# SnakeOnex/vit-is-all-you-need

Hardware: AMD Instinct MI355X
Metric: images/sec ViT-B/16 224px bf16 fwd+bwd (higher is better)
Workload: dtype bf16; 1 GPU; ViT-B/16 224x224 bf16 forward+loss+backward, batch 256 per GPU (BASELINE configs[1]; configs[2] at 8 GPUs), random-init weights, 197 tokens, 79.44 M params; global_batch=256, parallelism=dp1

## Files before the change

### vit-is-all-you-need_amd/csrc/gemm_nt_ld.h

```cpp
#pragma once
#include "gemm_nt_seam.h"

namespace {

template <int EPI, bool TAB = false, int SCHED = 1>
__global__ __launch_bounds__(768) void gemm_nt_ld_kernel(const GemmNtArgs p) {
  static_assert(EPI == EPI_BIAS_BF16 || EPI == EPI_GELU || EPI == EPI_DGELU || EPI == EPI_DGELU_NOCS, "epilogues of the loader form");
  static_assert(SCHED == 1, "request schedule");
  static_assert(!TAB || EPI == EPI_GELU, "table = GELU");
  constexpr bool DG = EPI == EPI_DGELU || EPI == EPI_DGELU_NOCS;
  constexpr bool CS = EPI == EPI_DGELU;
  constexpr int BM = 256, BN = 256, MT = 8, NT = 4;
  constexpr int AREG = 16384, ABUF = 32768, BBUF = 32768, BBASE = 2 * ABUF, OPS = BBASE + 2 * BBUF;
  constexpr int STG = 2048, TABOFF = OPS + 8 * STG;
  constexpr unsigned OOB = 0x80000000u;

  extern __shared__ __attribute__((aligned(16))) char smem[];
  const int tid = threadIdx.x, lane = tid & 63;
  const int wave = __builtin_amdgcn_readfirstlane(tid >> 6);
  const int tiles_n = (p.N + BN - 1) / BN, tiles_m = (p.M + BM - 1) / BM;
  const int ntiles = tiles_m * tiles_n;
  const int K = p.K;
  const int nkt = K / 64;
  auto coords = [&](int ti) { return nt_tile<BM>(ti, tiles_m, tiles_n); };

  if (wave >= 8) {
    const int l = wave - 8;
    const srd_t srdA = make_srd(p.A, (size_t)p.M * K * 2);
    const srd_t srdB = make_srd(p.B, (size_t)p.N * K * 2);
    const srd_t srdBias = make_srd(p.bias ? (const void*)p.bias : p.out, p.bias ? (size_t)p.N * 4 : 0);
    const unsigned ldsA = lds_addr(smem) + l * 4096;
    const unsigned ldsB = lds_addr(smem) + BBASE + l * 8192;
    unsigned voffA[2][4], voffB[8];
    auto offsets = [&](const NtTile& t) {
      const int r8 = lane >> 3;
      const unsigned chunk = (unsigned)(((lane & 7) ^ r8) * 16);
#pragma unroll
      for (int h = 0; h < 2; ++h)
#pragma unroll
        for (int i = 0; i < 4; ++i) {
          const int a = 4 * l + i;
          const int row = min(t.m0 + (a >> 3) * 128 + h * 64 + (a & 7) * 8 + r8, p.M - 1);
          voffA[h][i] = (unsigned)row * (unsigned)(K * 2) + chunk;
        }
#pragma unroll
      for (int i = 0; i < 8; ++i) {
        const int row = min(t.n0 + (8 * l + i) * 8 + r8, p.N - 1);
        voffB[i] = (unsigned)row * (unsigned)(K * 2) + chunk;
      }
    };
    bool live = true;
    unsigned so = 0u, par = 0u;
    auto request_b = [&](int i) {
      asm_glds16(srdB, ldsB + par * BBUF + i * 1024, live ? voffB[i] : OOB, so);
    };
    auto request_a = [&](int h, int i) {
      asm_glds16(srdA, ldsA + par * ABUF + h * AREG + i * 1024, live ? voffA[h][i] : OOB, so);
    };
    auto target = [&](int kt, bool lv) {
      live = lv;
      so = live ? (unsigned)kt * 128u : 0u;
      par = (unsigned)(kt & 1);
    };
    __builtin_amdgcn_s_setprio(3);
    int ti = blockIdx.x;
    NtTile cur = coords(ti);
    offsets(cur);
    int bias_n0 = cur.n0;
    target(0, true);
#pragma unroll
    for (int i = 0; i < 8; ++i) request_b(i);
#pragma unroll
    for (int i = 0; i < 4; ++i) request_a(0, i);
#pragma unroll
    for (int i = 0; i < 4; ++i) request_a(1, i);
    VITAMD_WAIT_VM(4);
    __builtin_amdgcn_s_barrier();
    for (;;) {
      const int ti_next = ti + (int)gridDim.x;
      const bool has_next = ti_next < ntiles;
      for (int kt = 0; kt < nkt; ++kt) {
        const bool last = kt + 1 == nkt;
        if (last && has_next) {
          cur = coords(ti_next);
          offsets(cur);
        }
        target(last ? 0 : kt + 1, !last || has_next);
        request_b(0); request_b(1); request_b(2);
        __builtin_amdgcn_s_barrier();
        request_b(3); request_b(4); request_b(5);
        VITAMD_WAIT_VM(6);
        __builtin_amdgcn_s_barrier();
        if constexpr (!DG) {
          if (kt == 0) {
            asm_glds4(srdBias, lds_addr(smem) + OPS + l * STG, (unsigned)(bias_n0 + l * 64 + lane) * 4u, 0u);
            asm_glds4(srdBias, lds_addr(smem) + OPS + (4 + l) * STG, (unsigned)(bias_n0 + l * 64 + lane) * 4u, 0u);
          }
        }
        request_b(6); request_b(7); request_a(0, 0);
        __builtin_amdgcn_s_barrier();
        request_a(0, 1); request_a(0, 2); request_a(0, 3);
        __builtin_amdgcn_s_barrier();
        request_a(1, 0); request_a(1, 1);
        __builtin_amdgcn_s_barrier();
        request_a(1, 2); request_a(1, 3);
        __builtin_amdgcn_s_barrier();
        __builtin_amdgcn_s_barrier();
        VITAMD_WAIT_VM(4);
        __builtin_amdgcn_s_barrier();
      }
      __builtin_amdgcn_s_barrier();
      if (!has_next) break;
      ti = ti_next;
      bias_n0 = cur.n0;
    }
    asm volatile("s_waitcnt vmcnt(0)" ::: "memory");
    return;
  }

  const int wm = wave >> 2, wn = wave & 3;
  const srd_t rsO = make_srd(p.out, (size_t)p.M * p.ldo * 2);
  const srd_t rsO2 = make_srd(EPI == EPI_GELU ? p.out2 : p.out, (size_t)p.M * p.ldo * 2);
  const srd_t srdAux = make_srd(DG ? p.aux : p.out, (size_t)p.M * p.ldo * 2);
  if constexpr (TAB) gelu_table_to_lds(p.gelu_tab, smem + TABOFF, tid);
  __builtin_amdgcn_s_barrier();
  asm volatile("" ::: "memory");
  for (int ti = blockIdx.x; ti < ntiles; ti += (int)gridDim.x) {
    const NtTile cur = coords(ti);
    if (wm == 1) __builtin_amdgcn_s_barrier();
    f32x4 acc[MT][NT];
#pragma unroll
    for (int i = 0; i < MT; ++i)
#pragma unroll
      for (int j = 0; j < NT; ++j) acc[i][j] = (f32x4){0.f, 0.f, 0.f, 0.f};
    {
      int l2 = (int)__builtin_amdgcn_mbcnt_hi(~0u, __builtin_amdgcn_mbcnt_lo(~0u, 0u));
      asm volatile("" : "+v"(l2));
      const char *rdA[2], *rdB[2];
      frag_bases(smem + wm * 8192, l2, rdA);
      frag_bases(smem + BBASE + wn * 8192, l2, rdB);
      bf16x8 bq[NT], af[4];
      auto ktile = [&](auto bufc) {
        constexpr int BUF = decltype(bufc)::value;
#pragma unroll
        for (int ph = 0; ph < 4; ++ph) {
          const int ks = ph >> 1, h = ph & 1;
          if (h == 0) {
#pragma unroll
            for (int j = 0; j < NT; ++j) bq[j] = *(const bf16x8*)(rdB[ks] + BUF * BBUF + j * 2048);
          }
#pragma unroll
          for (int ii = 0; ii < 4; ++ii) af[ii] = *(const bf16x8*)(rdA[ks] + BUF * ABUF + h * AREG + ii * 2048);
          __builtin_amdgcn_sched_barrier(0);
          __builtin_amdgcn_s_barrier();
          asm volatile("s_waitcnt lgkmcnt(0)" ::: "memory");
          __builtin_amdgcn_sched_barrier(0);
          __builtin_amdgcn_s_setprio(1);
#pragma unroll
          for (int ii = 0; ii < 4; ++ii)
#pragma unroll
            for (int j = 0; j < NT; ++j)
              acc[4 * h + ii][j] = __builtin_amdgcn_mfma_f32_16x16x32_bf16(bq[j], af[ii], acc[4 * h + ii][j], 0, 0, 0);
          __builtin_amdgcn_s_setprio(0);
          __builtin_amdgcn_sched_barrier(0);
          __builtin_amdgcn_s_barrier();
          asm volatile("" ::: "memory");
        }
      };
      for (int kt = 0; kt < nkt; kt += 2) {
        ktile(std::integral_constant<int, 0>{});
        ktile(std::integral_constant<int, 1>{});
      }
    }
    if (wm == 0) __builtin_amdgcn_s_barrier();

    int ln = (int)__builtin_amdgcn_mbcnt_hi(~0u, __builtin_amdgcn_mbcnt_lo(~0u, 0u));
    asm volatile("" : "+v"(ln));
    const int mloc = ln & 15, g = ln >> 4, rsub = ln >> 3, pc = ln & 7;
    char* const stg = smem + OPS + wave * STG;
    const int m0 = cur.m0, n0 = cur.n0;
    const int ncol = n0 + wn * 64 + 8 * (pc ^ rsub);
    const bool ncol_ok = ncol < p.N;
    const int mrow0 = m0 + wm * 128 + rsub;
    const unsigned obase = ncol_ok ? (unsigned)mrow0 * (unsigned)(p.ldo * 2) + (unsigned)ncol * 2u : OOB;
    const unsigned rstep = (unsigned)(p.ldo * 2) * 8u;
    u32x4 aux[DG ? 2 * MT : 1];
    u32x2 pk[DG ? MT : 1][NT];
    f32x4 bias4[NT];
    if constexpr (DG) {
#pragma unroll
      for (int i = 0; i < MT; ++i)
#pragma unroll
        for (int j = 0; j < NT; ++j) pk[i][j] = (u32x2){pack_bf16x2(acc[i][j][0], acc[i][j][1]), pack_bf16x2(acc[i][j][2], acc[i][j][3])};
#pragma unroll
      for (int it = 0; it < 2 * MT; ++it) aux[it] = asm_bload16(srdAux, mrow0 + 8 * it < p.M ? obase : OOB, rstep * (unsigned)it);
      static_assert(MT == 8, "16 pre-load registers named in one asm statement");
      asm volatile("s_waitcnt vmcnt(0)" : "+v"(aux[0]), "+v"(aux[1]), "+v"(aux[2]), "+v"(aux[3]), "+v"(aux[4]), "+v"(aux[5]), "+v"(aux[6]), "+v"(aux[7]), "+v"(aux[8]), "+v"(aux[9]), "+v"(aux[10]), "+v"(aux[11]), "+v"(aux[12]), "+v"(aux[13]), "+v"(aux[14]), "+v"(aux[15]) :: "memory");
    } else {
#pragma unroll
      for (int j = 0; j < NT; ++j)
#pragma unroll
        for (int r = 0; r < 4; ++r) bias4[j][r] = round_bf16(((const float*)stg)[16 * j + 4 * g + r]);
    }
    float cs[8];
#pragma unroll
    for (int c = 0; c < 8; ++c) cs[c] = 0.f;
#pragma unroll
    for (int i = 0; i < MT; ++i) {
#pragma unroll
      for (int j = 0; j < NT; ++j) {
        u32x2 o;
        if constexpr (DG) o = pk[i][j];
        else {
          const f32x4 v = acc[i][j] + bias4[j];
          o = (u32x2){pack_bf16x2(v[0], v[1]), pack_bf16x2(v[2], v[3])};
        }
        *(u32x2*)(stg + mloc * 128 + (((2 * j + (g >> 1)) ^ (mloc & 7)) << 4) + (g & 1) * 8) = o;
      }
#pragma unroll
      for (int h = 0; h < 2; ++h) {
        const u32x4 v = *(const u32x4*)(stg + (rsub + 8 * h) * 128 + pc * 16);
        const unsigned voff = mrow0 + 16 * i + 8 * h < p.M ? obase : OOB;
        const unsigned soff = rstep * (unsigned)(2 * i + h);
        if constexpr (EPI == EPI_BIAS_BF16) {
          asm_bstore16_nt(v, rsO, voff, soff);
        } else if constexpr (EPI == EPI_GELU) {
          u32x4 a, d = v;
          if constexpr (TAB) gelu_lookup8(v, smem + TABOFF, p.gelu_dg != 0, a, d);
          else
#pragma unroll
            for (int c = 0; c < 4; ++c) {
              float dlo, dhi;
              a[c] = pack_bf16x2(gelu_fwd_grad(bf16lo(v[c]), dlo), gelu_fwd_grad(bf16hi(v[c]), dhi));
              if (p.gelu_dg) d[c] = pack_bf16x2(dlo, dhi);
            }
          asm_bstore16_nt(d, rsO, voff, soff);
          asm_bstore16_nt(a, rsO2, voff, soff);
        } else {
          const u32x4 pz = aux[2 * i + h];
          u32x4 o;
#pragma unroll
          for (int c = 0; c < 4; ++c) {
            const float lo = round_bf16(bf16lo(v[c]) * bf16lo(pz[c]));
            const float hi = round_bf16(bf16hi(v[c]) * bf16hi(pz[c]));
            if constexpr (CS) { if (voff != OOB) { cs[2 * c] += lo; cs[2 * c + 1] += hi; } }
            o[c] = pack_bf16x2(lo, hi);
          }
          asm_bstore16_nt(o, rsO, voff, soff);
        }
      }
    }
    if constexpr (CS) {
#pragma unroll
      for (int bf = 1; bf < 8; bf <<= 1)
#pragma unroll
        for (int c = 0; c < 8; ++c) cs[c] += __shfl_xor(cs[c], 9 * bf, 64);
      float s = cs[0];
#pragma unroll
      for (int c = 1; c < 8; ++c) s = rsub == c ? cs[c] : s;
      atomicAdd(p.colsum + n0 + wn * 64 + 8 * (pc ^ rsub) + rsub, s);
    }
    asm volatile("s_waitcnt lgkmcnt(0)" ::: "memory");
  }
}

template <int EPI, bool TAB = false, int SCHED = 1>
int launch_ld(const GemmNtArgs& p, hipStream_t stream, int cus) {
  if (TAB && !p.gelu_tab) return VITAMD_ERR_ARG;
  return launch_tiles(gemm_nt_ld_kernel<EPI, TAB, SCHED>, p, stream, 256, 768, 160 * 1024, cus);
}

static bool ld_ok(const GemmNtArgs& p) { return seam_ok(p) && p.K % 128 == 0; }

}
```

Baseline: 9351 images/sec.

## Prefetch dGELU epilogue factors in loader waves and hand over through LDS

For the dGELU epilogue GEMM with K=768, the loader waves now issue the aux-factor loads during the final k-tiles of the main loop, using a fully unrolled compile-time schedule. They then pass the factors to the compute waves through the freed operand LDS buffers. Previously the compute waves loaded those factors from global memory in the epilogue and stalled on vmcnt(0). The cost is extra loader registers (32 u32x4), two more barrier rounds per tile, and a ds_bpermute rewrite of the colsum shuffle.

```diff
diff --git a/vit-is-all-you-need_amd/csrc/gemm_nt_ld.h b/vit-is-all-you-need_amd/csrc/gemm_nt_ld.h
--- a/vit-is-all-you-need_amd/csrc/gemm_nt_ld.h
+++ b/vit-is-all-you-need_amd/csrc/gemm_nt_ld.h
@@ -1,15 +1,31 @@
 #pragma once
+#include <utility>
 #include "gemm_nt_seam.h"
 
 namespace {
+
+
+template <int NKT> struct NtFactorPlan {
+  static constexpr int FA = 4, FKT0 = NKT - 1 - 32 / FA;
+  static constexpr bool fetches(int kt) { return NKT > 0 && kt >= FKT0 && kt <= NKT - 2; }
+  static constexpr int it(int j) { return 8 * (j >> 4) + (j & 7); }
+  static constexpr int w(int j) { return (j >> 3) & 1; }
+  static constexpr int reg(int j) { return 16 * w(j) + it(j); }
+};
+template <int... I, class F>
+__device__ __forceinline__ void nt_static_for(std::integer_sequence<int, I...>, F&& f) { (f(std::integral_constant<int, I>{}), ...); }
 
 template <int EPI, bool TAB = false, int SCHED = 1>
 __global__ __launch_bounds__(768) void gemm_nt_ld_kernel(const GemmNtArgs p) {
   static_assert(EPI == EPI_BIAS_BF16 || EPI == EPI_GELU || EPI == EPI_DGELU || EPI == EPI_DGELU_NOCS, "epilogues of the loader form");
-  static_assert(SCHED == 1, "request schedule");
+  constexpr int NKT = SCHED == 1 ? 0 : SCHED;
   static_assert(!TAB || EPI == EPI_GELU, "table = GELU");
   constexpr bool DG = EPI == EPI_DGELU || EPI == EPI_DGELU_NOCS;
   constexpr bool CS = EPI == EPI_DGELU;
+  constexpr bool PF = NKT > 0;
+  using FP = NtFactorPlan<NKT>;
+  constexpr int FA = FP::FA, FKT0 = FP::FKT0;
+  static_assert(!PF || (DG && NKT % 2 == 0 && FKT0 >= 0), "factor-prefetch form");
   constexpr int BM = 256, BN = 256, MT = 8, NT = 4;
   constexpr int AREG = 16384, ABUF = 32768, BBUF = 32768, BBASE = 2 * ABUF, OPS = BBASE + 2 * BBUF;
   constexpr int STG = 2048, TABOFF = OPS + 8 * STG;
@@ -21,8 +37,9 @@
   const int tiles_n = (p.N + BN - 1) / BN, tiles_m = (p.M + BM - 1) / BM;
   const int ntiles = tiles_m * tiles_n;
   const int K = p.K;
-  const int nkt = K / 64;
+  const int nkt = PF ? NKT : K / 64;
   auto coords = [&](int ti) { return nt_tile<BM>(ti, tiles_m, tiles_n); };
+  auto handover = [&](int w) { return smem + (w < 4 ? ABUF : BBASE + BBUF) + (w & 3) * 8192; };
 
   if (wave >= 8) {
     const int l = wave - 8;
@@ -32,9 +49,24 @@
     const unsigned ldsA = lds_addr(smem) + l * 4096;
     const unsigned ldsB = lds_addr(smem) + BBASE + l * 8192;
     unsigned voffA[2][4], voffB[8];
+    const srd_t srdAux = make_srd(DG ? p.aux : p.out, (size_t)p.M * p.ldo * 2);
+    u32x4 fr[PF ? 32 : 1];
+    unsigned fbase = OOB;
+    int frows = 0;
     auto offsets = [&](const NtTile& t) {
-      const int r8 = lane >> 3;
-      const unsigned chunk = (unsigned)(((lane & 7) ^ r8) * 16);
+      int ln = lane;
+      if constexpr (PF) {
+        ln = (int)__builtin_amdgcn_mbcnt_hi(~0u, __builtin_amdgcn_mbcnt_lo(~0u, 0u));
+        asm volatile("" : "+v"(ln));
+      }
+      const int r8 = ln >> 3;
+      const unsigned chunk = (unsigned)(((ln & 7) ^ r8) * 16);
+      if constexpr (PF) {
+        const int mrow0 = t.m0 + (l >> 1) * 128 + r8;
+        const int ncol = t.n0 + (2 * l & 3) * 64 + 8 * ((ln & 7) ^ r8);
+        fbase = ncol < p.N ? (unsigned)mrow0 * (unsigned)(p.ldo * 2) + (unsigned)ncol * 2u : OOB;
+        frows = p.M - mrow0;
+      }
 #pragma unroll
       for (int h = 0; h < 2; ++h)
 #pragma unroll
@@ -57,6 +89,7 @@
     auto request_a = [&](int h, int i) {
       asm_glds16(srdA, ldsA + par * ABUF + h * AREG + i * 1024, live ? voffA[h][i] : OOB, so);
     };
+    const unsigned rstep = (unsigned)(p.ldo * 2) * 8u;
     auto target = [&](int kt, bool lv) {
       live = lv;
       so = live ? (unsigned)kt * 128u : 0u;
@@ -79,6 +112,7 @@
     for (;;) {
       const int ti_next = ti + (int)gridDim.x;
       const bool has_next = ti_next < ntiles;
+      if constexpr (!PF) {
       for (int kt = 0; kt < nkt; ++kt) {
         const bool last = kt + 1 == nkt;
         if (last && has_next) {
@@ -109,7 +143,60 @@
         VITAMD_WAIT_VM(4);
         __builtin_amdgcn_s_barrier();
       }
+      } else {
+        nt_static_for(std::make_integer_sequence<int, PF ? NKT : 1>{}, [&](auto ktc) {
+          constexpr int KT = decltype(ktc)::value;
+          constexpr bool last = KT + 1 == NKT;
+          if (last && has_next) {
+            cur = coords(ti_next);
+            offsets(cur);
+          }
+          target(last ? 0 : KT + 1, !last || has_next);
+          request_b(0); request_b(1); request_b(2);
+          __builtin_amdgcn_s_barrier();
+          request_b(3); request_b(4); request_b(5);
+          VITAMD_WAIT_VM(FP::fetches(KT - 1) ? 6 + FA : 6);
+          __builtin_amdgcn_s_barrier();
+          request_b(6); request_b(7); request_a(0, 0);
+          __builtin_amdgcn_s_barrier();
+          request_a(0, 1); request_a(0, 2); request_a(0, 3);
+          __builtin_amdgcn_s_barrier();
+          request_a(1, 0); request_a(1, 1);
+          __builtin_amdgcn_s_barrier();
+          request_a(1, 2); request_a(1, 3);
+          __builtin_amdgcn_s_barrier();
+          __builtin_amdgcn_s_barrier();
+          if constexpr (FP::fetches(KT - 1)) {
+            constexpr int J = (KT - 1 - FKT0) * FA;
+            static_assert(FA == 4, "four factor registers named in one asm statement");
+            asm volatile("s_waitcnt vmcnt(4)" : "+v"(fr[FP::reg(J)]), "+v"(fr[FP::reg(J + 1)]), "+v"(fr[FP::reg(J + 2)]), "+v"(fr[FP::reg(J + 3)]) :: "memory");
+          } else {
+            VITAMD_WAIT_VM(4);
+          }
+          if constexpr (FP::fetches(KT)) {
+#pragma unroll
+            for (int a = 0; a < FA; ++a) {
+              const int j = (KT - FKT0) * FA + a, it = FP::it(j), w = FP::w(j);
+              fr[FP::reg(j)] = asm_bload16(srdAux, 8 * it < frows ? fbase : OOB, rstep * (unsigned)it + 128u * (unsigned)w);
+            }
+          }
+          __builtin_amdgcn_s_barrier();
+        });
+      }
       __builtin_amdgcn_s_barrier();
+      if constexpr (PF) {
+#pragma unroll
+        for (int half = 0; half < 2; ++half) {
+#pragma unroll
+          for (int w = 0; w < 2; ++w)
+#pragma unroll
+            for (int it = 0; it < 8; ++it) *(u32x4*)(handover(2 * l + w) + it * 1024 + lane * 16) = fr[16 * w + 8 * half + it];
+          asm volatile("s_waitcnt lgkmcnt(0)" ::: "memory");
+          __builtin_amdgcn_s_barrier();
+          __builtin_amdgcn_s_barrier();
+          asm volatile("" ::: "memory");
+        }
+      }
       if (!has_next) break;
       ti = ti_next;
       bias_n0 = cur.n0;
@@ -192,6 +279,18 @@
       for (int i = 0; i < MT; ++i)
 #pragma unroll
         for (int j = 0; j < NT; ++j) pk[i][j] = (u32x2){pack_bf16x2(acc[i][j][0], acc[i][j][1]), pack_bf16x2(acc[i][j][2], acc[i][j][3])};
+    }
+    if constexpr (PF) {
+#pragma unroll
+      for (int half = 0; half < 2; ++half) {
+        __builtin_amdgcn_s_barrier();
+        asm volatile("" ::: "memory");
+#pragma unroll
+        for (int it = 0; it < 8; ++it) aux[8 * half + it] = *(const u32x4*)(handover(wave) + it * 1024 + ln * 16);
+        asm volatile("s_waitcnt lgkmcnt(0)" ::: "memory");
+        __builtin_amdgcn_s_barrier();
+      }
+    } else if constexpr (DG) {
 #pragma unroll
       for (int it = 0; it < 2 * MT; ++it) aux[it] = asm_bload16(srdAux, mrow0 + 8 * it < p.M ? obase : OOB, rstep * (unsigned)it);
       static_assert(MT == 8, "16 pre-load registers named in one asm statement");
@@ -254,7 +353,10 @@
 #pragma unroll
       for (int bf = 1; bf < 8; bf <<= 1)
 #pragma unroll
-        for (int c = 0; c < 8; ++c) cs[c] += __shfl_xor(cs[c], 9 * bf, 64);
+        for (int c = 0; c < 8; ++c) {
+          if constexpr (PF) cs[c] += __builtin_bit_cast(float, __builtin_amdgcn_ds_bpermute((ln ^ (9 * bf)) << 2, __builtin_bit_cast(int, cs[c])));
+          else cs[c] += __shfl_xor(cs[c], 9 * bf, 64);
+        }
       float s = cs[0];
 #pragma unroll
       for (int c = 1; c < 8; ++c) s = rsub == c ? cs[c] : s;
@@ -267,6 +369,9 @@
 template <int EPI, bool TAB = false, int SCHED = 1>
 int launch_ld(const GemmNtArgs& p, hipStream_t stream, int cus) {
   if (TAB && !p.gelu_tab) return VITAMD_ERR_ARG;
+  if constexpr (EPI == EPI_DGELU || EPI == EPI_DGELU_NOCS) {
+    if (SCHED == 1 && p.K == 12 * 64) return launch_tiles(gemm_nt_ld_kernel<EPI, false, 12>, p, stream, 256, 768, 160 * 1024, cus);
+  }
   return launch_tiles(gemm_nt_ld_kernel<EPI, TAB, SCHED>, p, stream, 256, 768, 160 * 1024, cus);
 }
 
```

Result: no change. 9393 images/sec (median of 6 runs) (+0.4%).
